# VITA-Group/Open-L2O

Measured on NVIDIA H100. Metric: coordinate-updates/sec (N_params x unroll_steps), higher is better.
Workload: dtype f32

## Files before the change

include/l2o_b200.h:

```cpp
#ifndef L2O_B200_H_
#define L2O_B200_H_

#include <stddef.h>
#include <stdint.h>

#ifdef __cplusplus
extern "C" {
#endif

#define L2O_OK 0
#define L2O_E_INVALID (-1)
#define L2O_E_UNSUPPORTED (-2)
#define L2O_E_CUDA (-3)
#define L2O_E_NOMEM (-4)

#define L2O_PRE_IDENTITY 0
#define L2O_PRE_LOGSIGN 1
#define L2O_PRE_FC 2

#define L2O_OPT_NONE 0
#define L2O_OPT_RASTRIGIN_SEP 1
#define L2O_OPT_QUADRATIC_DIAG 2
#define L2O_OPT_QUADRATIC_BATCH 3

// ... 40 lines not shown
  const float* in_seq;
  int32_t opt_kind;
  const float* opt_a;
  const float* opt_b;
  float opt_alpha;
  float opt_fscale;
  float* x;
  float* state;
  float* ckpt;
  float* m;
  float* v;
  float beta1, beta2;
  int32_t step0;
  float* g_rec;
  float* feat_rec;
  double* fx;
  float* delta_seq;
  const float* labels;
  double* imit_loss;
  int64_t n_total;
  int32_t opt_group;
} l2o_unroll_args;

typedef struct {
  int64_t n;
  int32_t T;
  const float* theta;
  const float* in_seq;
  const float* ckpt;
  const float* g_rec;
  const float* labels;
  int64_t n_total;
  double* dtheta;
  const float* delta_seq;
  float* scratch;
} l2o_bwd_args;

int l2o_net_create(l2o_handle* out, const l2o_net_desc* desc);
void l2o_net_destroy(l2o_handle h);
int l2o_net_set_engine(l2o_handle h, int32_t engine);
int64_t l2o_theta_count(l2o_handle h);
int64_t l2o_state_floats(l2o_handle h);
int l2o_workspace_bytes(l2o_handle h, int64_t n, int32_t T, size_t* fwd_bytes, size_t* bwd_bytes);

typedef struct {
  float* d_state;
  float* lam;
} l2o_bwd_carry;

int l2o_step(l2o_handle h, const l2o_step_args* a, void* stream);
int l2o_unroll_fwd(l2o_handle h, const l2o_unroll_args* a, void* stream);
int l2o_unroll_bwd(l2o_handle h, const l2o_bwd_args* a, void* stream);
int l2o_unroll_bwd_carry(l2o_handle h, const l2o_bwd_args* a, const l2o_bwd_carry* c, void* stream);

int l2o_adam_step(float* theta, const double* dtheta, float* m, float* v, int64_t n, int32_t k, float lr,
                  float beta1, float beta2, float eps, void* stream);

int l2o_log_and_sign(const float* g, float* out, int64_t n, float k, void* stream);

typedef struct l2o_dense* l2o_dense_handle;
typedef struct {
  int32_t n_layers;
  int32_t hidden[2];
  int32_t n_in;
  int32_t preprocess;
  float logsign_k;
  int32_t n_out;
  float scale;
  int32_t tanh_output;
} l2o_dense_desc;
typedef struct {
  int64_t rows;
  const float* theta;
  const float* in;
  const float* state_in;
  float* state_out;
  float* x;
  float* delta;
} l2o_dense_step_args;
typedef struct {
  int64_t rows;
  int32_t T;
  const float* theta;
  const float* in_seq;
  const float* ckpt;
  const float* g_rec;
  const float* labels;
  int64_t n_total;
  double* dtheta;
} l2o_dense_bwd_args;
int l2o_dense_create(l2o_dense_handle* out, const l2o_dense_desc* desc);
void l2o_dense_destroy(l2o_dense_handle h);
int64_t l2o_dense_theta_count(l2o_dense_handle h);
int64_t l2o_dense_state_floats(l2o_dense_handle h);
int l2o_dense_step(l2o_dense_handle h, const l2o_dense_step_args* a, void* stream);
int l2o_dense_unroll_bwd(l2o_dense_handle h, const l2o_dense_bwd_args* a, void* stream);

typedef struct {
  int32_t batch, m, n;
  const float* A;
  const float* y;
  const float* x;
  const float* scale;
  float l1;
  float* g;
  double* f;
// ... 130 lines not shown
```

open_l2o_b200/_lib.py:

```python
from __future__ import annotations

import ctypes as C
import os
import subprocess
import sys

_HERE = os.path.dirname(os.path.abspath(__file__))
_ROOT = os.path.dirname(_HERE)
CSRC = os.path.join(_HERE, "csrc")
LIB_PATH = os.environ.get("L2O_LIB") or os.path.join(CSRC, "libl2o_b200.so")
INCLUDE = os.path.join(_ROOT, "include")

L2O_OK, L2O_E_INVALID, L2O_E_UNSUPPORTED, L2O_E_CUDA, L2O_E_NOMEM = 0, -1, -2, -3, -4
PRE_IDENTITY, PRE_LOGSIGN, PRE_FC = 0, 1, 2
OPT_NONE, OPT_RASTRIGIN_SEP, OPT_QUADRATIC_DIAG, OPT_QUADRATIC_BATCH = 0, 1, 2, 3
ENGINE_AUTO, ENGINE_FFMA, ENGINE_TC = 0, 1, 2

EXPORTS = [
    "l2o_net_create", "l2o_net_destroy", "l2o_net_set_engine", "l2o_theta_count", "l2o_state_floats", "l2o_workspace_bytes",
    "l2o_step", "l2o_unroll_fwd", "l2o_unroll_bwd", "l2o_unroll_bwd_carry", "l2o_adam_step", "l2o_log_and_sign", "l2o_lasso_grad",
    "l2o_dense_create", "l2o_dense_destroy", "l2o_dense_theta_count", "l2o_dense_state_floats", "l2o_dense_step",
    "l2o_dense_unroll_bwd",
    "l2o_launch_count", "l2o_status_string", "l2o_last_cuda_error", "l2o_version",
    "l2o_hrnn_create", "l2o_hrnn_destroy", "l2o_hrnn_theta_count", "l2o_hrnn_state_floats", "l2o_hrnn_coords",
    "l2o_hrnn_workspace_bytes", "l2o_hrnn_init_state", "l2o_hrnn_prepare", "l2o_hrnn_step",
    "l2o_hrnn_set_global_sizes", "l2o_hrnn_reduce_layout", "l2o_hrnn_prepare_local", "l2o_hrnn_prepare_finish",
    "l2o_hrnn_step_local", "l2o_hrnn_step_finish", "l2o_hrnn_coord_bwd", "l2o_hrnn_workspace_layout",
    "l2o_crnn_theta_count", "l2o_crnn_state_floats", "l2o_crnn_step", "l2o_crnn_bwd",
    "l2o_tadam_theta_count", "l2o_tadam_state_floats", "l2o_tadam_step", "l2o_tadam_bwd", "l2o_lrsgd_step",
    "l2o_lrsgd_bwd",
]


class NetDesc(C.Structure):
    _fields_ = [("n_layers", C.c_int32), ("hidden", C.c_int32 * 2), ("preprocess", C.c_int32),
                ("n_in", C.c_int32), ("fc_dim", C.c_int32), ("logsign_k", C.c_float), ("scale", C.c_float),
                ("tanh_output", C.c_int32)]


_fp = C.c_void_p


class StepArgs(C.Structure):
    _fields_ = [("n", C.c_int64), ("theta", _fp), ("in0", _fp), ("in1", _fp), ("m", _fp), ("v", _fp),
                ("beta1", C.c_float), ("beta2", C.c_float), ("p", C.c_float), ("state_in", _fp),
                ("state_out", _fp), ("x", _fp), ("delta", _fp), ("feat_out", _fp), ("step_ptr", _fp), ("t_offset", C.c_int32),
                ("reuse_weights", C.c_int32)]


class UnrollArgs(C.Structure):
    _fields_ = [("n", C.c_int64), ("T", C.c_int32), ("theta", _fp), ("in_seq", _fp), ("opt_kind", C.c_int32),
                ("opt_a", _fp), ("opt_b", _fp), ("opt_alpha", C.c_float), ("opt_fscale", C.c_float), ("x", _fp),
                ("state", _fp), ("ckpt", _fp), ("m", _fp), ("v", _fp), ("beta1", C.c_float), ("beta2", C.c_float),
                ("step0", C.c_int32), ("g_rec", _fp), ("feat_rec", _fp), ("fx", _fp), ("delta_seq", _fp),
                ("labels", _fp), ("imit_loss", _fp), ("n_total", C.c_int64), ("opt_group", C.c_int32)]


class BwdArgs(C.Structure):
    _fields_ = [("n", C.c_int64), ("T", C.c_int32), ("theta", _fp), ("in_seq", _fp), ("ckpt", _fp), ("g_rec", _fp),
                ("labels", _fp), ("n_total", C.c_int64), ("dtheta", _fp), ("delta_seq", _fp), ("scratch", _fp)]


class BwdCarry(C.Structure):
    _fields_ = [("d_state", _fp), ("lam", _fp)]


class LassoArgs(C.Structure):
    _fields_ = [("batch", C.c_int32), ("m", C.c_int32), ("n", C.c_int32), ("A", _fp), ("y", _fp), ("x", _fp),
                ("scale", _fp), ("l1", C.c_float), ("g", _fp), ("f", _fp)]


class DenseDesc(C.Structure):
    _fields_ = [("n_layers", C.c_int32), ("hidden", C.c_int32 * 2), ("n_in", C.c_int32), ("preprocess", C.c_int32),
# ... 85 lines not shown
            return None
        cmd = ["nvcc"] + NVCC_FLAGS + ["-c", "-o", obj, tu]
        if verbose:
            print(" ".join(cmd), file=sys.stderr)
        r = subprocess.run(cmd, capture_output=True, text=True)
        if r.returncode != 0:
            raise L2OError("nvcc failed for %s:\n%s%s" % (tu, r.stdout, r.stderr))
        return obj

    with ThreadPoolExecutor(max_workers=max(1, min(len(jobs), os.cpu_count() or 1))) as ex:
        rebuilt = [o for o in ex.map(compile_one, jobs) if o]
    objs = [j[1] for j in jobs]
    if rebuilt or not os.path.exists(LIB_PATH) or os.path.getmtime(LIB_PATH) < max(os.path.getmtime(o) for o in objs):
        cmd = ["nvcc"] + ARCH + ["-shared", "-o", LIB_PATH] + objs
        if verbose:
            print(" ".join(cmd), file=sys.stderr)
        r = subprocess.run(cmd, capture_output=True, text=True)
        if r.returncode != 0:
            raise L2OError("link failed:\n" + r.stdout + r.stderr)
    return LIB_PATH


_lib = None


def lib():
    global _lib
    if _lib is not None:
        return _lib
    if not os.path.exists(LIB_PATH):
        raise L2OError(f"{LIB_PATH} not found - run `python -c 'import __graft_entry__ as g; g.build()'` "
                       "(there is no CPU/PyTorch fallback)")
    L = C.CDLL(LIB_PATH)
    L.l2o_net_create.argtypes = [C.POINTER(C.c_void_p), C.POINTER(NetDesc)]
    L.l2o_net_create.restype = C.c_int
    L.l2o_net_destroy.argtypes = [C.c_void_p]
    L.l2o_net_destroy.restype = None
    L.l2o_net_set_engine.argtypes = [C.c_void_p, C.c_int32]
    L.l2o_net_set_engine.restype = C.c_int
    L.l2o_theta_count.argtypes = [C.c_void_p]
    L.l2o_theta_count.restype = C.c_int64
    L.l2o_state_floats.argtypes = [C.c_void_p]
    L.l2o_state_floats.restype = C.c_int64
    L.l2o_workspace_bytes.argtypes = [C.c_void_p, C.c_int64, C.c_int32, C.POINTER(C.c_size_t), C.POINTER(C.c_size_t)]
    L.l2o_workspace_bytes.restype = C.c_int
    L.l2o_step.argtypes = [C.c_void_p, C.POINTER(StepArgs), C.c_void_p]
    L.l2o_step.restype = C.c_int
    L.l2o_unroll_fwd.argtypes = [C.c_void_p, C.POINTER(UnrollArgs), C.c_void_p]
    L.l2o_unroll_fwd.restype = C.c_int
    L.l2o_unroll_bwd.argtypes = [C.c_void_p, C.POINTER(BwdArgs), C.c_void_p]
    L.l2o_unroll_bwd.restype = C.c_int
    L.l2o_unroll_bwd_carry.argtypes = [C.c_void_p, C.POINTER(BwdArgs), C.POINTER(BwdCarry), C.c_void_p]
    L.l2o_unroll_bwd_carry.restype = C.c_int
    L.l2o_adam_step.argtypes = [C.c_void_p, C.c_void_p, C.c_void_p, C.c_void_p, C.c_int64, C.c_int32, C.c_float,
                                C.c_float, C.c_float, C.c_float, C.c_void_p]
    L.l2o_adam_step.restype = C.c_int
    L.l2o_log_and_sign.argtypes = [C.c_void_p, C.c_void_p, C.c_int64, C.c_float, C.c_void_p]
    L.l2o_log_and_sign.restype = C.c_int
    L.l2o_lasso_grad.argtypes = [C.POINTER(LassoArgs), C.c_void_p]
    L.l2o_lasso_grad.restype = C.c_int
    L.l2o_dense_create.argtypes = [C.POINTER(C.c_void_p), C.POINTER(DenseDesc)]
    L.l2o_dense_create.restype = C.c_int
    L.l2o_dense_destroy.argtypes = [C.c_void_p]
    L.l2o_dense_destroy.restype = None
    for name in ("l2o_dense_theta_count", "l2o_dense_state_floats"):
        getattr(L, name).argtypes = [C.c_void_p]
        getattr(L, name).restype = C.c_int64
    L.l2o_dense_step.argtypes = [C.c_void_p, C.POINTER(DenseStepArgs), C.c_void_p]
    L.l2o_dense_step.restype = C.c_int
    L.l2o_dense_unroll_bwd.argtypes = [C.c_void_p, C.POINTER(DenseBwdArgs), C.c_void_p]
    L.l2o_dense_unroll_bwd.restype = C.c_int
    L.l2o_launch_count.argtypes = []
    L.l2o_launch_count.restype = C.c_int64
    L.l2o_hrnn_create.argtypes = [C.POINTER(C.c_void_p), C.POINTER(C.c_int64), C.c_int32]
    L.l2o_hrnn_create.restype = C.c_int
    L.l2o_hrnn_destroy.argtypes = [C.c_void_p]
    L.l2o_hrnn_destroy.restype = None
    L.l2o_hrnn_theta_count.argtypes = []
    L.l2o_hrnn_theta_count.restype = C.c_int64
    L.l2o_hrnn_state_floats.argtypes = []
    L.l2o_hrnn_state_floats.restype = C.c_int64
    for name in ("l2o_hrnn_coords", "l2o_hrnn_workspace_bytes"):
        getattr(L, name).argtypes = [C.c_void_p]
        getattr(L, name).restype = C.c_int64
    L.l2o_hrnn_set_global_sizes.argtypes = [C.c_void_p, C.POINTER(C.c_int64)]
    L.l2o_hrnn_set_global_sizes.restype = C.c_int
    L.l2o_hrnn_reduce_layout.argtypes = [C.c_void_p, C.POINTER(C.c_int64), C.POINTER(C.c_int64), C.POINTER(C.c_int64)]
    L.l2o_hrnn_reduce_layout.restype = C.c_int
    L.l2o_hrnn_coord_bwd.argtypes = [C.c_void_p, C.POINTER(HrnnBwdArgs), C.c_void_p]
    L.l2o_hrnn_coord_bwd.restype = C.c_int
    L.l2o_hrnn_workspace_layout.argtypes = [C.c_void_p, C.POINTER(C.c_int64)]
    L.l2o_hrnn_workspace_layout.restype = C.c_int
    for name in ("l2o_hrnn_init_state", "l2o_hrnn_prepare", "l2o_hrnn_step", "l2o_hrnn_prepare_local",
                 "l2o_hrnn_prepare_finish", "l2o_hrnn_step_local", "l2o_hrnn_step_finish"):
        getattr(L, name).argtypes = [C.c_void_p, C.POINTER(HrnnArgs), C.c_void_p]
        getattr(L, name).restype = C.c_int
    for name in ("l2o_crnn_theta_count", "l2o_crnn_state_floats"):
        getattr(L, name).argtypes = []
        getattr(L, name).restype = C.c_int64
    L.l2o_crnn_step.argtypes = [C.POINTER(CrnnStepArgs), C.c_void_p]
    L.l2o_crnn_step.restype = C.c_int
    L.l2o_crnn_bwd.argtypes = [C.POINTER(CrnnBwdArgs), C.c_void_p]
    L.l2o_crnn_bwd.restype = C.c_int
    for name in ("l2o_tadam_theta_count", "l2o_tadam_state_floats"):
        getattr(L, name).argtypes = []
        getattr(L, name).restype = C.c_int64
# ... 19 lines not shown
```

open_l2o_b200/csrc/cwlstm_tc.cuh:

```cuda
#pragma once
#include "cwlstm_common.cuh"

namespace l2o {
namespace tc {

constexpr int kH = 20;
constexpr int kN = 4 * kH;
constexpr int kTile = 64;
constexpr int kU = 5;
constexpr int kFwdWG = 3;
constexpr int kFwdThreads = 128 * kFwdWG;
template <int N>
struct IC {
  static constexpr int value = N;
};

template <class C>
struct Geo {
  static constexpr bool FC = C::FC;
  static constexpr int ColH1 = FC ? 24 : 4, ColH2 = FC ? 44 : 24;
  static constexpr int ColOne = FC ? 20 : C::F;
  static constexpr int KB = FC ? 8 : 6;
  static constexpr int L1Lo = 0, L1Hi = FC ? 6 : 3;
  static constexpr int L2Lo = FC ? 2 : 0, L2Hi = KB;
// ... 217 lines not shown
    mma_rs<N>(d, f.hi[kb], bl + o, 1u);
    mma_rs<N>(d, f.hi[kb], bh + o, 1u);
  }
}

__host__ __device__ constexpr int acc_idx(int s, int g, int rh) { return 4 * (2 * s + (g >> 1)) + 2 * rh + (g & 1); }

constexpr float kLog2e = 1.4426950408889634f;
__device__ __forceinline__ void lstm_point_fwd(float zi, float zj, float zf, float zo, float& c, float& h) {
  const float Ei = ex2_approx(fminf(-kLog2e * zi, 40.f));
  const float Ej = ex2_approx(fminf(-2.f * kLog2e * zj, 40.f));
  const float Qf = 1.0f + ex2_approx(fminf(fmaf(-kLog2e, zf, -kLog2e), 40.f));
  const float Pij = (1.0f + Ei) * (1.0f + Ej);
  const float cn = fmaf(c, Pij, (1.0f - Ej) * Qf) * rcp_approx(Pij * Qf);
  c = cn;
  const float Ec = ex2_approx(fminf(-2.f * kLog2e * cn, 63.f));
  const float Eo = ex2_approx(fminf(-kLog2e * zo, 63.f));
  h = (1.0f - Ec) * rcp_approx((1.0f + Ec) * (1.0f + Eo));
}
__device__ __forceinline__ float elu_fast(float av) {
  const float em = ex2_approx(kLog2e * av) - 1.0f;
  const float ep = av * fmaf(av, fmaf(av, fmaf(av, 1.0f / 24.0f, 1.0f / 6.0f), 0.5f), 1.0f);
  return av > 0.f ? av : (av > -0.0625f ? ep : em);
}

__device__ __forceinline__ void load5(const float* __restrict__ p, int q, float* v) {
#pragma unroll
  for (int s = 0; s < kU; ++s) v[s] = p[5 * q + s];
}
__device__ __forceinline__ void store5(float* __restrict__ p, int q, const float* v) {
#pragma unroll
  for (int s = 0; s < kU; ++s) p[5 * q + s] = v[s];
}
__device__ __forceinline__ float quad_sum(float v) {
  v += __shfl_xor_sync(0xffffffffu, v, 1);
  return v + __shfl_xor_sync(0xffffffffu, v, 2);
}
__device__ __forceinline__ float from_row(float v, int lane, int rh) {
  return __shfl_sync(0xffffffffu, v, (lane & ~3) | rh);
}

struct FwdExtra {
  const int32_t* step_ptr;
  int32_t t_offset;
  float p_fixed;
};

template <class C>
struct SmemF {
  float img[Geo<C>::FwdFloats];
  float wo[kH + 4];
  float win[64];
  uint64_t wbar;
  uint64_t pad;
  double fx[1];
};
template <class C>
__host__ __device__ constexpr size_t adamc_offset(int T) {
  return (sizeof(SmemF<C>) + (size_t)(T + 1) * sizeof(double) + 15) & ~(size_t)15;
}
template <class C>
__host__ __device__ constexpr size_t fwd_smem_bytes(int T) {
  return adamc_offset<C>(T) + (C::FC ? (size_t)T * 2 * sizeof(float) : 0);
}

template <class C>
__global__ void __launch_bounds__(kFwdThreads, 1) unroll_fwd_kernel(l2o_unroll_args a, NetRt rt, const float* __restrict__ img,
                                                                     float* __restrict__ state_out, FwdExtra ex) {
  using G = Geo<C>;
  extern __shared__ __align__(128) unsigned char smem_raw[];
  SmemF<C>& S = *reinterpret_cast<SmemF<C>*>(smem_raw);
  const int T = a.T;
  const int64_t n = a.n;
  const bool in_kernel_opt = a.opt_kind != L2O_OPT_NONE;
  const bool want_fx = in_kernel_opt && a.fx != nullptr;
  const bool adam_mode = C::NIN == 2 && a.m != nullptr;
  float* adamc = reinterpret_cast<float*>(smem_raw + adamc_offset<C>(T));

  if (want_fx)
    for (int t = threadIdx.x; t <= T; t += blockDim.x) S.fx[t] = 0.0;
  if (threadIdx.x < kH) S.wo[threadIdx.x] = a.theta[C::O_WO + threadIdx.x];
  if (threadIdx.x == kH) S.wo[kH] = a.theta[C::O_BO];
  if constexpr (C::FC) {
    static_assert(!C::FC || C::NIN == 2, "fc nets here are RNNprop nets (two inputs)");
    if (threadIdx.x >= 32 && threadIdx.x < 92) S.win[threadIdx.x - 32] = a.theta[C::O_WIN + threadIdx.x - 32];
    if (adam_mode) {
      const int step0 = ex.step_ptr ? *ex.step_ptr + ex.t_offset : a.step0;
      for (int t = threadIdx.x; t < T; t += blockDim.x) {
        const float p = (ex.step_ptr == nullptr && ex.p_fixed > 0.f) ? ex.p_fixed : (float)(step0 + t);
        adamc[2 * t] = 1.0f - powf(a.beta1, p);
        adamc[2 * t + 1] = 1.0f - powf(a.beta2, p);
      }
    }
  }
  if (threadIdx.x == 0) {
    mbar_init(&S.wbar, 1);
    fence_barrier_init();
  }
  __syncthreads();
  stage_image(S.img, img, G::FwdFloats * 4, &S.wbar);

  const int wg = threadIdx.x >> 7, warp = (threadIdx.x >> 5) & 3, lane = threadIdx.x & 31;
  const int g = lane >> 2, q = lane & 3, own = q & 1;
  const uint64_t b1h = img_desc(S.img, kN), b1l = img_desc(S.img + G::B1Floats, kN);
  const uint64_t b2h = img_desc(S.img + 2 * G::B1Floats, kN), b2l = img_desc(S.img + 2 * G::B1Floats + G::B2Floats, kN);
  const int64_t ntiles = (n + kTile - 1) / kTile;
  const int64_t slot = n * C::SF;
  const float bo = S.wo[kH];
  float wo[kU];
#pragma unroll
  for (int s = 0; s < kU; ++s) wo[s] = S.wo[5 * q + s];
  double imit = 0.0;
  float d[kN / 2];
#pragma unroll
  for (int k = 0; k < kN / 2; ++k) d[k] = 0.f;

  for (int64_t tile = (int64_t)blockIdx.x * kFwdWG + wg; tile < ntiles; tile += (int64_t)gridDim.x * kFwdWG) {
    const int64_t r0 = tile * kTile + warp * 16 + g;
    const int64_t row[2] = {r0, r0 + 8};
    const bool act[2] = {row[0] < n, row[1] < n};
    const int64_t io = own ? row[1] : row[0];
    const bool oact = io < n;
    const bool writer = q < 2 && oact;
    Frag<G::KB> A;
    A.zero();
    float c1[2][kU], c2[2][kU];
#pragma unroll
    for (int rh = 0; rh < 2; ++rh) {
      float h1[kU] = {0.f, 0.f, 0.f, 0.f, 0.f}, h2[kU] = {0.f, 0.f, 0.f, 0.f, 0.f};
#pragma unroll
      for (int s = 0; s < kU; ++s) { c1[rh][s] = 0.f; c2[rh][s] = 0.f; }
      if (act[rh]) {
        const int64_t i = row[rh];
        load5(a.state + i * kH, q, h1);
        load5(a.state + (n + i) * kH, q, c1[rh]);
        load5(a.state + 2 * n * kH + i * kH, q, h2);
        load5(a.state + 2 * n * kH + (n + i) * kH, q, c2[rh]);
        if (a.ckpt) {
          store5(a.ckpt + i * kH, q, h1);
          store5(a.ckpt + (n + i) * kH, q, c1[rh]);
          store5(a.ckpt + 2 * n * kH + i * kH, q, h2);
          store5(a.ckpt + 2 * n * kH + (n + i) * kH, q, c2[rh]);
        }
        if (T == 0 && state_out != a.state) {
          store5(state_out + i * kH, q, h1);
          store5(state_out + (n + i) * kH, q, c1[rh]);
          store5(state_out + 2 * n * kH + i * kH, q, h2);
          store5(state_out + 2 * n * kH + (n + i) * kH, q, c2[rh]);
        }
      }
      A.template put_vec<G::ColH1>(rh, h1);
      A.template put_vec<G::ColH2>(rh, h2);
    }
    if constexpr (G::FC) {
      A.template put<G::ColOne>(0, q == 0 ? 1.0f : 0.f);
      A.template put<G::ColOne>(1, q == 0 ? 1.0f : 0.f);
    }
    float x = 0.f, oa = 0.f, ob = 0.f, am = 0.f, av = 0.f;
    if (oact) {
      if (a.x) x = a.x[io];
      if (in_kernel_opt) { oa = a.opt_a[io]; ob = a.opt_b[io]; }
      if (adam_mode) { am = a.m[io]; av = a.v[io]; }
    }

    for (int t = 0; t < T; ++t) {
      float fval = 0.f, raw0 = 0.f, raw1 = 0.f;
      if (oact) {
        if (in_kernel_opt) {
          optimizee_eval(a.opt_kind, x, oa, ob, a.opt_alpha, a.opt_fscale, fval, raw0);
          if (a.g_rec && q < 2) a.g_rec[(int64_t)t * n + io] = raw0;
        } else if (C::NIN == 2 && !adam_mode) {
          raw0 = a.in_seq[((int64_t)t * 2) * n + io];
          raw1 = a.in_seq[((int64_t)t * 2 + 1) * n + io];
        } else {
          raw0 = a.in_seq[(int64_t)t * n + io];
        }
      }
      if constexpr (G::FC) {
        if (adam_mode) {
          const float gg = raw0;
          am = a.beta1 * am + (1.0f - a.beta1) * gg;
          av = a.beta2 * av + (1.0f - a.beta2) * gg * gg;
          const float mh = am / adamc[2 * t], vh = av / adamc[2 * t + 1];
          const float den = sqrtf(vh) + 1e-8f;
          raw0 = mh / den;
          raw1 = gg / den;
        }
        if (writer && a.feat_rec) {
          a.feat_rec[((int64_t)t * 2) * n + io] = raw0;
          a.feat_rec[((int64_t)t * 2 + 1) * n + io] = raw1;
        }
#pragma unroll
        for (int rh = 0; rh < 2; ++rh) {
          const float m0 = from_row(raw0, lane, rh), m1 = from_row(raw1, lane, rh);
          float u[kU];
#pragma unroll
          for (int s = 0; s < kU; ++s) {
            const int j = 5 * q + s;
            u[s] = elu_fast(fmaf(m1, S.win[kH + j], fmaf(m0, S.win[j], S.win[2 * kH + j])));
          }
          A.template put_vec<0>(rh, u);
        }
      } else {
        float f[C::F];
        preprocess<C>(nullptr, rt, raw0, raw1, f);
#pragma unroll
        for (int rh = 0; rh < 2; ++rh) {
          float v = q == C::F ? 1.0f : 0.f;
#pragma unroll
          for (int k = 0; k < C::F; ++k) {
            const float fk = from_row(f[k], lane, rh);
            if (q == k) v = fk;
          }
          A.template put<0>(rh, v);
        }
      }
      if (want_fx) {
        const double ws = warp_sum_d(q < 2 ? (double)fval : 0.0);
        if (lane == 0) atomicAdd(&S.fx[t], ws);
      }
      wg_fence();
      mma3<kN, G::KB, G::L1Lo, G::L1Hi>(d, A, b1h, b1l);
      wg_commit();
      wg_wait<0>();
#pragma unroll
      for (int rh = 0; rh < 2; ++rh) {
        float h[kU];
#pragma unroll
        for (int s = 0; s < kU; ++s)
          lstm_point_fwd(d[acc_idx(s, 0, rh)], d[acc_idx(s, 1, rh)], d[acc_idx(s, 2, rh)], d[acc_idx(s, 3, rh)], c1[rh][s], h[s]);
        A.template put_vec<G::ColH1>(rh, h);
        if (act[rh]) {
          const int64_t i = row[rh];
          if (a.ckpt) {
            float* ck = a.ckpt + (int64_t)(t + 1) * slot;
            store5(ck + i * kH, q, h);
            store5(ck + (n + i) * kH, q, c1[rh]);
          }
          if (t == T - 1) {
            store5(state_out + i * kH, q, h);
            store5(state_out + (n + i) * kH, q, c1[rh]);
          }
        }
      }
      wg_fence();
      mma3<kN, G::KB, G::L2Lo, G::L2Hi>(d, A, b2h, b2l);
      wg_commit();
      wg_wait<0>();
      float y[2];
#pragma unroll
      for (int rh = 0; rh < 2; ++rh) {
        float h[kU];
        float yp = 0.f;
#pragma unroll
        for (int s = 0; s < kU; ++s) {
          lstm_point_fwd(d[acc_idx(s, 0, rh)], d[acc_idx(s, 1, rh)], d[acc_idx(s, 2, rh)], d[acc_idx(s, 3, rh)], c2[rh][s], h[s]);
          yp = fmaf(h[s], wo[s], yp);
        }
        A.template put_vec<G::ColH2>(rh, h);
        y[rh] = quad_sum(yp) + bo;
        if (act[rh]) {
          const int64_t i = row[rh];
          if (a.ckpt) {
            float* ck = a.ckpt + (int64_t)(t + 1) * slot + 2 * n * kH;
            store5(ck + i * kH, q, h);
            store5(ck + (n + i) * kH, q, c2[rh]);
          }
          if (t == T - 1) {
            store5(state_out + 2 * n * kH + i * kH, q, h);
            store5(state_out + 2 * n * kH + (n + i) * kH, q, c2[rh]);
          }
        }
      }
      const float yo = own ? y[1] : y[0];
      const float dl = rt.tanh_output ? tanh_acc(yo) * rt.scale : yo * rt.scale;
      x += dl;
      if (writer) {
        if (a.delta_seq) a.delta_seq[(int64_t)t * n + io] = dl;
        if (a.labels) {
          const float r = a.labels[(int64_t)t * n + io] - dl;
          imit += 0.5 * (double)r * (double)r;
        }
      }
    }
    float fval = 0.f;
    if (writer) {
      if (in_kernel_opt) {
        float gT;
        optimizee_eval(a.opt_kind, x, oa, ob, a.opt_alpha, a.opt_fscale, fval, gT);
        if (a.g_rec) a.g_rec[(int64_t)T * n + io] = gT;
      }
      if (a.x) a.x[io] = x;
      if (adam_mode) { a.m[io] = am; a.v[io] = av; }
    }
    if (want_fx) {
      const double ws = warp_sum_d((double)fval);
      if (lane == 0) atomicAdd(&S.fx[T], ws);
    }
  }
  if (a.labels && a.imit_loss) {
    const double ws = warp_sum_d(imit);
    if (lane == 0) atomicAdd(a.imit_loss, ws / (double)a.n_total);
  }
  __syncthreads();
  if (want_fx)
    for (int t = threadIdx.x; t <= T; t += blockDim.x) atomicAdd(&a.fx[t], S.fx[t]);
}

}

template <class C>
int tc_launch_fwd(const NetRt& rt, const l2o_unroll_args& a, float* img, cudaStream_t st, int sms, float* state_out = nullptr,
                  tc::FwdExtra ex = tc::FwdExtra{nullptr, 0, 0.f}, bool prep = true) {
  if (prep) tc::prep_weights_kernel<C><<<16, 256, 0, st>>>(a.theta, img, 0);
  auto k = tc::unroll_fwd_kernel<C>;
  const size_t smem = tc::fwd_smem_bytes<C>(a.T);
  if (smem > 227 * 1024) return L2O_E_INVALID;
  if (cudaFuncSetAttribute(k, cudaFuncAttributeMaxDynamicSharedMemorySize, (int)smem) != cudaSuccess) return L2O_E_CUDA;
  const int64_t ntiles = (a.n + tc::kTile - 1) / tc::kTile;
  const int64_t ctas = (ntiles + tc::kFwdWG - 1) / tc::kFwdWG;
  const int grid = (int)(ctas < sms ? ctas : sms);
  k<<<grid, tc::kFwdThreads, smem, st>>>(a, rt, img, state_out ? state_out : a.state, ex);
  return cudaGetLastError() == cudaSuccess ? L2O_OK : L2O_E_CUDA;
}

}
```

open_l2o_b200/csrc/l2o_capi.cu:

```cuda
#include <cuda_runtime.h>

#include <atomic>
#include <cmath>
#include <cstdio>
#include <new>

#include "l2o_internal.h"

namespace {
std::atomic<int64_t> g_launches{0};
thread_local char g_cuda_err[256] = "";

int find_cfg(const l2o_net_desc& d) {
  const int h1 = d.n_layers >= 1 ? d.hidden[0] : 0;
  const int h2 = d.n_layers >= 2 ? d.hidden[1] : 0;
  const int f = d.preprocess == L2O_PRE_FC ? d.fc_dim : (d.preprocess == L2O_PRE_LOGSIGN ? 2 * d.n_in : d.n_in);
#define X(id, PRE, NIN, F, H1, H2) \
  if (d.preprocess == PRE && d.n_in == NIN && f == F && h1 == H1 && h2 == H2) return id;
  L2O_FOR_EACH_CFG(X)
#undef X
  return -1;
}

__global__ void adam_kernel(float* __restrict__ theta, const double* __restrict__ dtheta, float* __restrict__ m,
// ... 80 lines not shown
  h->engine = engine;
  return L2O_OK;
}

int64_t l2o_theta_count(l2o_handle h) { return h ? h->n_theta : L2O_E_INVALID; }
int64_t l2o_state_floats(l2o_handle h) { return h ? h->state_floats : L2O_E_INVALID; }

int l2o_workspace_bytes(l2o_handle h, int64_t n, int32_t T, size_t* fwd_bytes, size_t* bwd_bytes) {
  if (!h || n < 0 || T < 0) return L2O_E_INVALID;
  const size_t arena = (size_t)h->state_floats * (size_t)n * sizeof(float);
  const size_t ckpt = arena * ((size_t)T + 1);
  const size_t grec = (size_t)(T + 1) * (size_t)n * sizeof(float);
  const size_t feat = h->desc.n_in == 2 ? (size_t)T * 2 * (size_t)n * sizeof(float) : 0;
  if (fwd_bytes) *fwd_bytes = arena + ckpt + grec + feat;
  const size_t fc_extra = h->cfg == 2 ? (size_t)T * (size_t)n * (1 + 20) * sizeof(float) : 0;
  if (bwd_bytes) *bwd_bytes = ckpt + grec + feat + fc_extra + (size_t)h->n_theta * sizeof(double);
  return L2O_OK;
}

int l2o_step(l2o_handle h, const l2o_step_args* a, void* stream) {
  if (!h || !a || a->n < 0 || !a->theta || !a->in0) return L2O_E_INVALID;
  if (h->state_floats > 0 && (!a->state_in || !a->state_out)) return L2O_E_INVALID;
  if (h->desc.n_in == 2 && !a->m && !a->in1) return L2O_E_INVALID;
  if ((a->m == nullptr) != (a->v == nullptr)) return L2O_E_INVALID;
  if (a->m && h->desc.n_in != 2) return L2O_E_INVALID;
  if (a->n == 0) return L2O_OK;
  cudaStream_t st = (cudaStream_t)stream;
  const bool tc_can = l2o::tc_step_ok(h, *a);
  if (h->engine == L2O_ENGINE_TC) return tc_can ? l2o::tc_step(h, *a, st) : L2O_E_UNSUPPORTED;
  if (h->engine == L2O_ENGINE_AUTO && tc_can && l2o::tc_auto_default() && a->n >= 16384) return l2o::tc_step(h, *a, st);
  return l2o::ffma_step(h, *a, st);
}

int l2o_unroll_fwd(l2o_handle h, const l2o_unroll_args* a, void* stream) {
  if (!h || !a || a->n < 0 || a->T < 0 || !a->theta) return L2O_E_INVALID;
  if (a->opt_kind == L2O_OPT_NONE && !a->in_seq && a->T > 0) return L2O_E_INVALID;
  if (a->opt_kind < L2O_OPT_NONE || a->opt_kind > L2O_OPT_QUADRATIC_BATCH) return L2O_E_INVALID;
  if (a->opt_kind == L2O_OPT_QUADRATIC_BATCH &&
      (a->opt_group < 1 || a->opt_group > 128 || a->n % a->opt_group != 0)) return L2O_E_INVALID;
  if (a->opt_kind != L2O_OPT_NONE && (!a->x || !a->opt_a || !a->opt_b)) return L2O_E_INVALID;
  if (a->opt_kind != L2O_OPT_NONE && h->desc.n_in == 2 && !a->m) return L2O_E_INVALID;
  if (h->state_floats > 0 && !a->state) return L2O_E_INVALID;
  if ((a->m == nullptr) != (a->v == nullptr)) return L2O_E_INVALID;
  if (a->m && h->desc.n_in != 2) return L2O_E_INVALID;
  if (a->labels && (!a->imit_loss || a->n_total <= 0)) return L2O_E_INVALID;
  if (a->n == 0) return L2O_OK;
  cudaStream_t st = (cudaStream_t)stream;
  const bool tc_can = l2o::tc_supported(h->cfg) && l2o::tc_fwd_ok(h, *a);
  if (h->engine == L2O_ENGINE_TC) return tc_can ? l2o::tc_unroll_fwd(h, *a, st) : L2O_E_UNSUPPORTED;
  if (h->engine == L2O_ENGINE_AUTO && tc_can && l2o::tc_auto_default()) return l2o::tc_unroll_fwd(h, *a, st);
  return l2o::ffma_unroll_fwd(h, *a, st);
}

int l2o_unroll_bwd(l2o_handle h, const l2o_bwd_args* a, void* stream) {
  if (!h || !a || a->n < 0 || a->T < 0 || !a->theta || !a->dtheta) return L2O_E_INVALID;
  if (a->T > 0 && !a->in_seq) return L2O_E_INVALID;
  if (h->state_floats > 0 && !a->ckpt) return L2O_E_INVALID;
  if (reinterpret_cast<uintptr_t>(a->ckpt) % 16 != 0) return L2O_E_INVALID;
  if (!a->g_rec && (!a->labels || a->n_total <= 0)) return L2O_E_INVALID;
  if (a->n == 0 || a->T == 0) return L2O_OK;
  cudaStream_t st = (cudaStream_t)stream;
  const bool tc_can = l2o::tc_bwd_ok(h, *a);
  if (h->engine == L2O_ENGINE_TC) return tc_can ? l2o::tc_unroll_bwd(h, *a, st) : L2O_E_UNSUPPORTED;
  if (h->engine == L2O_ENGINE_AUTO && tc_can && l2o::tc_bwd_auto_default()) return l2o::tc_unroll_bwd(h, *a, st);
  return l2o::ffma_unroll_bwd(h, *a, st);
}

int l2o_unroll_bwd_carry(l2o_handle h, const l2o_bwd_args* a, const l2o_bwd_carry* c, void* stream) {
  if (!h || !a || !c || a->n < 0 || a->T < 0 || !a->theta || !a->dtheta) return L2O_E_INVALID;
  if (a->T > 0 && !a->in_seq) return L2O_E_INVALID;
  if (h->state_floats > 0 && (!a->ckpt || !c->d_state)) return L2O_E_INVALID;
  if (reinterpret_cast<uintptr_t>(a->ckpt) % 16 != 0 || reinterpret_cast<uintptr_t>(c->d_state) % 16 != 0)
    return L2O_E_INVALID;
  if (!c->lam) return L2O_E_INVALID;
  if (!a->g_rec && (!a->labels || a->n_total <= 0)) return L2O_E_INVALID;
  if (a->labels) return L2O_E_UNSUPPORTED;
  if (a->n == 0 || a->T == 0) return L2O_OK;
  cudaStream_t st = (cudaStream_t)stream;
  const bool tc_can = l2o::tc_bwd_ok(h, *a);
  if (h->engine == L2O_ENGINE_TC) return tc_can ? l2o::tc_unroll_bwd(h, *a, st, c) : L2O_E_UNSUPPORTED;
  if (h->engine == L2O_ENGINE_AUTO && tc_can && l2o::tc_bwd_auto_default()) return l2o::tc_unroll_bwd(h, *a, st, c);
  return l2o::ffma_unroll_bwd(h, *a, st, c);
}

int l2o_adam_step(float* theta, const double* dtheta, float* m, float* v, int64_t n, int32_t k, float lr, float beta1,
                  float beta2, float eps, void* stream) {
  if (!theta || !dtheta || !m || !v || n < 0 || k < 1) return L2O_E_INVALID;
  if (n == 0) return L2O_OK;
  const double lr_t = (double)lr * std::sqrt(1.0 - std::pow((double)beta2, k)) / (1.0 - std::pow((double)beta1, k));
  const int block = 256;
  adam_kernel<<<(int)((n + block - 1) / block), block, 0, (cudaStream_t)stream>>>(theta, dtheta, m, v, n, (float)lr_t,
                                                                                 beta1, beta2, eps);
  l2o::count_launch();
  L2O_CUDA_TRY(cudaGetLastError());
  return L2O_OK;
}

int l2o_log_and_sign(const float* g, float* out, int64_t n, float k, void* stream) {
  if (!g || !out || n < 0) return L2O_E_INVALID;
  if (n == 0) return L2O_OK;
  const int block = 256;
  log_and_sign_kernel<<<(int)((n + block - 1) / block), block, 0, (cudaStream_t)stream>>>(g, out, n, k,
                                                                                         (float)std::exp((double)k));
  l2o::count_launch();
  L2O_CUDA_TRY(cudaGetLastError());
  return L2O_OK;
// ... 20 lines not shown
```

open_l2o_b200/csrc/l2o_internal.h:

```cpp
#pragma once
#include <cuda_runtime.h>

#include "cwlstm_common.cuh"
#include "l2o_b200.h"

#define L2O_FOR_EACH_CFG(X)               \
  X(0, L2O_PRE_IDENTITY, 1, 1, 20, 20)    \
  X(1, L2O_PRE_LOGSIGN, 1, 2, 20, 20)     \
  X(2, L2O_PRE_FC, 2, 20, 20, 20)         \
  X(3, L2O_PRE_IDENTITY, 1, 1, 0, 0)      \
  X(4, L2O_PRE_IDENTITY, 1, 1, 1, 0)      \
  X(5, L2O_PRE_IDENTITY, 1, 1, 1, 1)      \
  X(6, L2O_PRE_IDENTITY, 1, 1, 2, 3)

struct l2o_net {
  l2o_net_desc desc;
  int cfg;
  int engine;
  int64_t n_theta;
  int64_t state_floats;
  l2o::NetRt rt;
  float* tc_img;
  int tc_img_dev;
  int tc_img_mode;
};

namespace l2o {
int set_cuda_error(cudaError_t e, const char* where);
void count_launch(int n = 1);
int device_sms();

inline bool overlaps_any(const void* p, size_t bytes, const void* const* q, const size_t* qbytes, int nq) {
  const uintptr_t a = (uintptr_t)p;
  for (int k = 0; k < nq; ++k) {
    const uintptr_t b = (uintptr_t)q[k];
    if (b && a < b + qbytes[k] && b < a + bytes) return true;
  }
  return false;
}

int ffma_step(const l2o_net* h, const l2o_step_args& a, cudaStream_t st);
int ffma_unroll_fwd(const l2o_net* h, const l2o_unroll_args& a, cudaStream_t st);
int ffma_unroll_bwd(const l2o_net* h, const l2o_bwd_args& a, cudaStream_t st, const l2o_bwd_carry* c = nullptr);

bool tc_supported(int cfg);
void tc_release_image(l2o_net* h);
bool tc_fwd_ok(const l2o_net* h, const l2o_unroll_args& a);
int tc_unroll_fwd(l2o_net* h, const l2o_unroll_args& a, cudaStream_t st);
bool tc_step_ok(const l2o_net* h, const l2o_step_args& a);
int tc_step(l2o_net* h, const l2o_step_args& a, cudaStream_t st);
bool tc_auto_default();
bool tc_bwd_auto_default();
bool tc_bwd_ok(const l2o_net* h, const l2o_bwd_args& a);
int tc_unroll_bwd(l2o_net* h, const l2o_bwd_args& a, cudaStream_t st, const l2o_bwd_carry* c = nullptr);
}

#define L2O_CUDA_TRY(expr)                                              \
  do {                                                                  \
    cudaError_t e__ = (expr);                                           \
    if (e__ != cudaSuccess) return l2o::set_cuda_error(e__, #expr);     \
  } while (0)
```

open_l2o_b200/csrc/l2o_tc.cu:

```cuda
#include "cwlstm_ffma.cuh"
#include "cwlstm_tc.cuh"
#include "cwlstm_tc_bwd.cuh"
#include <cstdlib>
#include <mutex>
#include <utility>
#include <vector>
#include "l2o_internal.h"

namespace l2o {
bool tc_supported(int cfg) { return cfg == 0 || cfg == 1 || cfg == 2; }
bool tc_fwd_ok(const l2o_net* h, const l2o_unroll_args& a) {
  if (a.opt_kind == L2O_OPT_QUADRATIC_BATCH) return false;
  if (h->cfg == 2) return true;
  return a.m == nullptr && a.feat_rec == nullptr;
}
static bool tc_auto_env() {
  static const bool on = !(std::getenv("L2O_TC_AUTO") != nullptr && std::getenv("L2O_TC_AUTO")[0] == '0');
  return on;
}
bool tc_auto_default() { return tc_auto_env(); }
bool tc_bwd_auto_default() { return tc_auto_env(); }

namespace {
struct ImgPool {
// ... 70 lines not shown
  return tc_supported(h->cfg) && a.m == nullptr && a.in1 == nullptr && a.feat_out == nullptr;
}

int tc_step(l2o_net* h, const l2o_step_args& s, cudaStream_t st) {
  if (!tc_step_ok(h, s)) return L2O_E_UNSUPPORTED;
  int rc = ensure_image(h);
  if (rc) return rc;
  const int sms = device_sms();
  if (sms <= 0) return L2O_E_CUDA;
  l2o_unroll_args a{};
  a.n = s.n;
  a.T = 1;
  a.theta = s.theta;
  a.in_seq = s.in0;
  a.opt_kind = L2O_OPT_NONE;
  a.x = s.x;
  a.state = const_cast<float*>(s.state_in);
  a.delta_seq = s.delta;
  a.m = s.m;
  a.v = s.v;
  a.beta1 = s.beta1;
  a.beta2 = s.beta2;
  a.step0 = 1;
  a.feat_rec = s.feat_out;
  const tc::FwdExtra ex{s.step_ptr, s.t_offset, s.step_ptr ? 0.f : s.p};
  rc = L2O_E_UNSUPPORTED;
  const bool prep = !(s.reuse_weights && h->tc_img_mode == 0);
  if (h->cfg == 0) rc = tc_launch_fwd<Cfg<L2O_PRE_IDENTITY, 1, 1, 20, 20>>(h->rt, a, h->tc_img, st, sms, s.state_out, ex, prep);
  if (h->cfg == 1) rc = tc_launch_fwd<Cfg<L2O_PRE_LOGSIGN, 1, 2, 20, 20>>(h->rt, a, h->tc_img, st, sms, s.state_out, ex, prep);
  if (h->cfg == 2) rc = tc_launch_fwd<Cfg<L2O_PRE_FC, 2, 20, 20, 20>>(h->rt, a, h->tc_img, st, sms, s.state_out, ex, prep);
  if (rc == L2O_OK) count_launch(prep ? 2 : 1);
  h->tc_img_mode = 0;
  if (rc == L2O_E_CUDA) return set_cuda_error(cudaGetLastError(), "tc_step launch");
  return rc;
}

int tc_unroll_fwd(l2o_net* h, const l2o_unroll_args& a, cudaStream_t st) {
  if (!tc_supported(h->cfg) || !tc_fwd_ok(h, a)) return L2O_E_UNSUPPORTED;
  {
    int rc0 = ensure_image(h);
    if (rc0) return rc0;
  }
  const int sms = device_sms();
  if (sms <= 0) return L2O_E_CUDA;
  int rc = L2O_E_UNSUPPORTED;
  if (h->cfg == 0) rc = tc_launch_fwd<Cfg<L2O_PRE_IDENTITY, 1, 1, 20, 20>>(h->rt, a, h->tc_img, st, sms);
  if (h->cfg == 1) rc = tc_launch_fwd<Cfg<L2O_PRE_LOGSIGN, 1, 2, 20, 20>>(h->rt, a, h->tc_img, st, sms);
  if (h->cfg == 2) rc = tc_launch_fwd<Cfg<L2O_PRE_FC, 2, 20, 20, 20>>(h->rt, a, h->tc_img, st, sms);
  if (rc == L2O_OK) count_launch(2);
  h->tc_img_mode = 0;
  if (rc == L2O_E_CUDA) return set_cuda_error(cudaGetLastError(), "tc_unroll_fwd launch");
  return rc;
}
}
```

Measured before the change: 1.845 billion.

## Add specialized full-tile tensor-core forward for DM nets with in-kernel optimizee

Templates the forward unroll kernel on a FAST flag, optimizee kind and checkpoint presence, so that when n is a multiple of the tile size and no tanh, delta, or label outputs are requested, row-bound checks and runtime branches compile away. Final state is now written once after the time loop instead of inside it under a t==T-1 test. Checkpoint and g_rec addressing becomes incremental pointers. The per-step fx reduction goes straight to global atomics instead of a shared-memory buffer, and a query entry point reports which variant would run. The cost is more kernel instantiations, and more global atomic traffic on fx.

```diff
diff --git a/include/l2o_b200.h b/include/l2o_b200.h
--- a/include/l2o_b200.h
+++ b/include/l2o_b200.h
@@ -116,6 +116,7 @@
 int l2o_unroll_fwd(l2o_handle h, const l2o_unroll_args* a, void* stream);
 int l2o_unroll_bwd(l2o_handle h, const l2o_bwd_args* a, void* stream);
 int l2o_unroll_bwd_carry(l2o_handle h, const l2o_bwd_args* a, const l2o_bwd_carry* c, void* stream);
+int l2o_tc_fwd_variant(l2o_handle h, const l2o_unroll_args* a);
 
 int l2o_adam_step(float* theta, const double* dtheta, float* m, float* v, int64_t n, int32_t k, float lr,
                   float beta1, float beta2, float eps, void* stream);
diff --git a/open_l2o_b200/_lib.py b/open_l2o_b200/_lib.py
--- a/open_l2o_b200/_lib.py
+++ b/open_l2o_b200/_lib.py
@@ -18,7 +18,7 @@
 
 EXPORTS = [
     "l2o_net_create", "l2o_net_destroy", "l2o_net_set_engine", "l2o_theta_count", "l2o_state_floats", "l2o_workspace_bytes",
-    "l2o_step", "l2o_unroll_fwd", "l2o_unroll_bwd", "l2o_unroll_bwd_carry", "l2o_adam_step", "l2o_log_and_sign", "l2o_lasso_grad",
+    "l2o_step", "l2o_unroll_fwd", "l2o_unroll_bwd", "l2o_unroll_bwd_carry", "l2o_tc_fwd_variant", "l2o_adam_step", "l2o_log_and_sign", "l2o_lasso_grad",
     "l2o_dense_create", "l2o_dense_destroy", "l2o_dense_theta_count", "l2o_dense_state_floats", "l2o_dense_step",
     "l2o_dense_unroll_bwd",
     "l2o_launch_count", "l2o_status_string", "l2o_last_cuda_error", "l2o_version",
@@ -210,6 +210,8 @@
     L.l2o_unroll_bwd.restype = C.c_int
     L.l2o_unroll_bwd_carry.argtypes = [C.c_void_p, C.POINTER(BwdArgs), C.POINTER(BwdCarry), C.c_void_p]
     L.l2o_unroll_bwd_carry.restype = C.c_int
+    L.l2o_tc_fwd_variant.argtypes = [C.c_void_p, C.POINTER(UnrollArgs)]
+    L.l2o_tc_fwd_variant.restype = C.c_int
     L.l2o_adam_step.argtypes = [C.c_void_p, C.c_void_p, C.c_void_p, C.c_void_p, C.c_int64, C.c_int32, C.c_float,
                                 C.c_float, C.c_float, C.c_float, C.c_void_p]
     L.l2o_adam_step.restype = C.c_int
diff --git a/open_l2o_b200/csrc/cwlstm_tc.cuh b/open_l2o_b200/csrc/cwlstm_tc.cuh
--- a/open_l2o_b200/csrc/cwlstm_tc.cuh
+++ b/open_l2o_b200/csrc/cwlstm_tc.cuh
@@ -293,33 +293,42 @@
   float wo[kH + 4];
   float win[64];
   uint64_t wbar;
-  uint64_t pad;
-  double fx[1];
 };
 template <class C>
-__host__ __device__ constexpr size_t adamc_offset(int T) {
-  return (sizeof(SmemF<C>) + (size_t)(T + 1) * sizeof(double) + 15) & ~(size_t)15;
+__host__ __device__ constexpr size_t adamc_offset() {
+  return (sizeof(SmemF<C>) + 15) & ~(size_t)15;
 }
 template <class C>
 __host__ __device__ constexpr size_t fwd_smem_bytes(int T) {
-  return adamc_offset<C>(T) + (C::FC ? (size_t)T * 2 * sizeof(float) : 0);
-}
-
-template <class C>
+  return adamc_offset<C>() + (C::FC ? (size_t)T * 2 * sizeof(float) : 0);
+}
+__device__ __forceinline__ double warp_sum_pairs_d(double v) {
+  v += __shfl_xor_sync(0xffffffffu, v, 16);
+  v += __shfl_xor_sync(0xffffffffu, v, 8);
+  v += __shfl_xor_sync(0xffffffffu, v, 4);
+  return v + __shfl_xor_sync(0xffffffffu, v, 1);
+}
+
+template <class C, bool FAST = false, int OPT = L2O_OPT_NONE, bool CKPT = false>
 __global__ void __launch_bounds__(kFwdThreads, 1) unroll_fwd_kernel(l2o_unroll_args a, NetRt rt, const float* __restrict__ img,
                                                                      float* __restrict__ state_out, FwdExtra ex) {
+  static_assert(!FAST || (!C::FC && OPT != L2O_OPT_NONE), "the full-tile forward is the DM nets' with an optimizee");
   using G = Geo<C>;
   extern __shared__ __align__(128) unsigned char smem_raw[];
   SmemF<C>& S = *reinterpret_cast<SmemF<C>*>(smem_raw);
   const int T = a.T;
   const int64_t n = a.n;
-  const bool in_kernel_opt = a.opt_kind != L2O_OPT_NONE;
+  const bool in_kernel_opt = FAST || a.opt_kind != L2O_OPT_NONE;
+  const int opt_kind = FAST ? OPT : a.opt_kind;
   const bool want_fx = in_kernel_opt && a.fx != nullptr;
   const bool adam_mode = C::NIN == 2 && a.m != nullptr;
-  float* adamc = reinterpret_cast<float*>(smem_raw + adamc_offset<C>(T));
-
-  if (want_fx)
-    for (int t = threadIdx.x; t <= T; t += blockDim.x) S.fx[t] = 0.0;
+  const bool has_ckpt = FAST ? CKPT : a.ckpt != nullptr;
+  const bool has_grec = FAST ? CKPT : a.g_rec != nullptr;
+  const bool tanh_out = !FAST && rt.tanh_output;
+  const bool has_delta = !FAST && a.delta_seq != nullptr;
+  const bool has_labels = !FAST && a.labels != nullptr;
+  float* adamc = reinterpret_cast<float*>(smem_raw + adamc_offset<C>());
+
   if (threadIdx.x < kH) S.wo[threadIdx.x] = a.theta[C::O_WO + threadIdx.x];
   if (threadIdx.x == kH) S.wo[kH] = a.theta[C::O_BO];
   if constexpr (C::FC) {
@@ -341,12 +350,13 @@
   __syncthreads();
   stage_image(S.img, img, G::FwdFloats * 4, &S.wbar);
 
-  const int wg = threadIdx.x >> 7, warp = (threadIdx.x >> 5) & 3, lane = threadIdx.x & 31;
+  const int wg = __shfl_sync(0xffffffffu, threadIdx.x >> 7, 0), warp = (threadIdx.x >> 5) & 3, lane = threadIdx.x & 31;
   const int g = lane >> 2, q = lane & 3, own = q & 1;
   const uint64_t b1h = img_desc(S.img, kN), b1l = img_desc(S.img + G::B1Floats, kN);
   const uint64_t b2h = img_desc(S.img + 2 * G::B1Floats, kN), b2l = img_desc(S.img + 2 * G::B1Floats + G::B2Floats, kN);
   const int64_t ntiles = (n + kTile - 1) / kTile;
   const int64_t slot = n * C::SF;
+  const int64_t nk = n * kH;
   const float bo = S.wo[kH];
   float wo[kU];
 #pragma unroll
@@ -359,10 +369,12 @@
   for (int64_t tile = (int64_t)blockIdx.x * kFwdWG + wg; tile < ntiles; tile += (int64_t)gridDim.x * kFwdWG) {
     const int64_t r0 = tile * kTile + warp * 16 + g;
     const int64_t row[2] = {r0, r0 + 8};
-    const bool act[2] = {row[0] < n, row[1] < n};
+    const bool act[2] = {FAST || row[0] < n, FAST || row[1] < n};
     const int64_t io = own ? row[1] : row[0];
-    const bool oact = io < n;
+    const bool oact = FAST || io < n;
     const bool writer = q < 2 && oact;
+    float* ck = has_ckpt ? a.ckpt + r0 * kH : nullptr;
+    float* gr = has_grec ? a.g_rec + io : nullptr;
     Frag<G::KB> A;
     A.zero();
     float c1[2][kU], c2[2][kU];
@@ -377,13 +389,14 @@
         load5(a.state + (n + i) * kH, q, c1[rh]);
         load5(a.state + 2 * n * kH + i * kH, q, h2);
         load5(a.state + 2 * n * kH + (n + i) * kH, q, c2[rh]);
-        if (a.ckpt) {
-          store5(a.ckpt + i * kH, q, h1);
-          store5(a.ckpt + (n + i) * kH, q, c1[rh]);
-          store5(a.ckpt + 2 * n * kH + i * kH, q, h2);
-          store5(a.ckpt + 2 * n * kH + (n + i) * kH, q, c2[rh]);
-        }
-        if (T == 0 && state_out != a.state) {
+        if (has_ckpt) {
+          float* p = ck + rh * 8 * kH;
+          store5(p, q, h1);
+          store5(p + nk, q, c1[rh]);
+          store5(p + 2 * nk, q, h2);
+          store5(p + 3 * nk, q, c2[rh]);
+        }
+        if (!FAST && T == 0 && state_out != a.state) {
           store5(state_out + i * kH, q, h1);
           store5(state_out + (n + i) * kH, q, c1[rh]);
           store5(state_out + 2 * n * kH + i * kH, q, h2);
@@ -399,17 +412,21 @@
     }
     float x = 0.f, oa = 0.f, ob = 0.f, am = 0.f, av = 0.f;
     if (oact) {
-      if (a.x) x = a.x[io];
+      if (FAST || a.x) x = a.x[io];
       if (in_kernel_opt) { oa = a.opt_a[io]; ob = a.opt_b[io]; }
       if (adam_mode) { am = a.m[io]; av = a.v[io]; }
     }
 
     for (int t = 0; t < T; ++t) {
+      if (has_ckpt) ck += slot;
       float fval = 0.f, raw0 = 0.f, raw1 = 0.f;
       if (oact) {
         if (in_kernel_opt) {
-          optimizee_eval(a.opt_kind, x, oa, ob, a.opt_alpha, a.opt_fscale, fval, raw0);
-          if (a.g_rec && q < 2) a.g_rec[(int64_t)t * n + io] = raw0;
+          optimizee_eval(opt_kind, x, oa, ob, a.opt_alpha, a.opt_fscale, fval, raw0);
+          if (has_grec) {
+            if (q < 2) *gr = raw0;
+            gr += n;
+          }
         } else if (C::NIN == 2 && !adam_mode) {
           raw0 = a.in_seq[((int64_t)t * 2) * n + io];
           raw1 = a.in_seq[((int64_t)t * 2 + 1) * n + io];
@@ -457,8 +474,8 @@
         }
       }
       if (want_fx) {
-        const double ws = warp_sum_d(q < 2 ? (double)fval : 0.0);
-        if (lane == 0) atomicAdd(&S.fx[t], ws);
+        const double ws = warp_sum_pairs_d(q < 2 ? (double)fval : 0.0);
+        if (lane == 0) atomicAdd(&a.fx[t], ws);
       }
       wg_fence();
       mma3<kN, G::KB, G::L1Lo, G::L1Hi>(d, A, b1h, b1l);
@@ -471,18 +488,11 @@
         for (int s = 0; s < kU; ++s)
           lstm_point_fwd(d[acc_idx(s, 0, rh)], d[acc_idx(s, 1, rh)], d[acc_idx(s, 2, rh)], d[acc_idx(s, 3, rh)], c1[rh][s], h[s]);
         A.template put_vec<G::ColH1>(rh, h);
-        if (act[rh]) {
-          const int64_t i = row[rh];
-          if (a.ckpt) {
-            float* ck = a.ckpt + (int64_t)(t + 1) * slot;
-            store5(ck + i * kH, q, h);
-            store5(ck + (n + i) * kH, q, c1[rh]);
-          }
-          if (t == T - 1) {
-            store5(state_out + i * kH, q, h);
-            store5(state_out + (n + i) * kH, q, c1[rh]);
-          }
-        }
+        if (act[rh] && has_ckpt) {
+          store5(ck + rh * 8 * kH, q, h);
+          store5(ck + nk + rh * 8 * kH, q, c1[rh]);
+        }
+        if (has_ckpt) __syncwarp();
       }
       wg_fence();
       mma3<kN, G::KB, G::L2Lo, G::L2Hi>(d, A, b2h, b2l);
@@ -500,61 +510,73 @@
         }
         A.template put_vec<G::ColH2>(rh, h);
         y[rh] = quad_sum(yp) + bo;
-        if (act[rh]) {
-          const int64_t i = row[rh];
-          if (a.ckpt) {
-            float* ck = a.ckpt + (int64_t)(t + 1) * slot + 2 * n * kH;
-            store5(ck + i * kH, q, h);
-            store5(ck + (n + i) * kH, q, c2[rh]);
-          }
-          if (t == T - 1) {
-            store5(state_out + 2 * n * kH + i * kH, q, h);
-            store5(state_out + 2 * n * kH + (n + i) * kH, q, c2[rh]);
-          }
-        }
+        if (act[rh] && has_ckpt) {
+          store5(ck + 2 * nk + rh * 8 * kH, q, h);
+          store5(ck + 3 * nk + rh * 8 * kH, q, c2[rh]);
+        }
+        if (has_ckpt) __syncwarp();
       }
       const float yo = own ? y[1] : y[0];
-      const float dl = rt.tanh_output ? tanh_acc(yo) * rt.scale : yo * rt.scale;
+      const float dl = tanh_out ? tanh_acc(yo) * rt.scale : __fmul_rn(yo, rt.scale);
       x += dl;
       if (writer) {
-        if (a.delta_seq) a.delta_seq[(int64_t)t * n + io] = dl;
-        if (a.labels) {
+        if (has_delta) a.delta_seq[(int64_t)t * n + io] = dl;
+        if (has_labels) {
           const float r = a.labels[(int64_t)t * n + io] - dl;
           imit += 0.5 * (double)r * (double)r;
         }
+      }
+    }
+    if (FAST || T > 0) {
+#pragma unroll
+      for (int rh = 0; rh < 2; ++rh) {
+        if (!act[rh]) continue;
+        float h1[kU], h2[kU];
+#pragma unroll
+        for (int s = 0; s < kU; ++s) {
+          h1[s] = A.get_at(G::ColH1 + 4 * s, rh);
+          h2[s] = A.get_at(G::ColH2 + 4 * s, rh);
+        }
+        float* p = state_out + row[rh] * kH;
+        store5(p, q, h1);
+        store5(p + nk, q, c1[rh]);
+        store5(p + 2 * nk, q, h2);
+        store5(p + 3 * nk, q, c2[rh]);
       }
     }
     float fval = 0.f;
     if (writer) {
       if (in_kernel_opt) {
         float gT;
-        optimizee_eval(a.opt_kind, x, oa, ob, a.opt_alpha, a.opt_fscale, fval, gT);
-        if (a.g_rec) a.g_rec[(int64_t)T * n + io] = gT;
-      }
-      if (a.x) a.x[io] = x;
+        optimizee_eval(opt_kind, x, oa, ob, a.opt_alpha, a.opt_fscale, fval, gT);
+        if (has_grec) *gr = gT;
+      }
+      if (FAST || a.x) a.x[io] = x;
       if (adam_mode) { a.m[io] = am; a.v[io] = av; }
     }
     if (want_fx) {
-      const double ws = warp_sum_d((double)fval);
-      if (lane == 0) atomicAdd(&S.fx[T], ws);
-    }
-  }
-  if (a.labels && a.imit_loss) {
+      const double ws = warp_sum_pairs_d((double)fval);
+      if (lane == 0) atomicAdd(&a.fx[T], ws);
+    }
+  }
+  if (has_labels && a.imit_loss) {
     const double ws = warp_sum_d(imit);
     if (lane == 0) atomicAdd(a.imit_loss, ws / (double)a.n_total);
   }
-  __syncthreads();
-  if (want_fx)
-    for (int t = threadIdx.x; t <= T; t += blockDim.x) atomicAdd(&a.fx[t], S.fx[t]);
-}
-
-}
-
-template <class C>
-int tc_launch_fwd(const NetRt& rt, const l2o_unroll_args& a, float* img, cudaStream_t st, int sms, float* state_out = nullptr,
-                  tc::FwdExtra ex = tc::FwdExtra{nullptr, 0, 0.f}, bool prep = true) {
-  if (prep) tc::prep_weights_kernel<C><<<16, 256, 0, st>>>(a.theta, img, 0);
-  auto k = tc::unroll_fwd_kernel<C>;
+}
+
+}
+
+inline bool tc_fwd_fast(bool fc, const NetRt& rt, const l2o_unroll_args& a, const float* state_out) {
+  return !fc && (a.opt_kind == L2O_OPT_RASTRIGIN_SEP || a.opt_kind == L2O_OPT_QUADRATIC_DIAG) && a.n > 0 &&
+         a.n % tc::kTile == 0 && a.T > 0 && (state_out == nullptr || state_out == a.state) && a.x != nullptr &&
+         (a.ckpt == nullptr) == (a.g_rec == nullptr) && !rt.tanh_output && a.delta_seq == nullptr && a.labels == nullptr;
+}
+
+template <class C, bool FAST, int OPT, bool CKPT>
+int tc_run_fwd(const NetRt& rt, const l2o_unroll_args& a, float* img, cudaStream_t st, int sms, float* state_out,
+               tc::FwdExtra ex) {
+  auto k = tc::unroll_fwd_kernel<C, FAST, OPT, CKPT>;
   const size_t smem = tc::fwd_smem_bytes<C>(a.T);
   if (smem > 227 * 1024) return L2O_E_INVALID;
   if (cudaFuncSetAttribute(k, cudaFuncAttributeMaxDynamicSharedMemorySize, (int)smem) != cudaSuccess) return L2O_E_CUDA;
@@ -565,4 +587,21 @@
   return cudaGetLastError() == cudaSuccess ? L2O_OK : L2O_E_CUDA;
 }
 
-}
+template <class C>
+int tc_launch_fwd(const NetRt& rt, const l2o_unroll_args& a, float* img, cudaStream_t st, int sms, float* state_out = nullptr,
+                  tc::FwdExtra ex = tc::FwdExtra{nullptr, 0, 0.f}, bool prep = true) {
+  if (prep) tc::prep_weights_kernel<C><<<16, 256, 0, st>>>(a.theta, img, 0);
+  if constexpr (!C::FC) {
+    if (tc_fwd_fast(false, rt, a, state_out)) {
+      constexpr int R = L2O_OPT_RASTRIGIN_SEP, Q = L2O_OPT_QUADRATIC_DIAG;
+      if (a.opt_kind == R)
+        return a.ckpt ? tc_run_fwd<C, true, R, true>(rt, a, img, st, sms, state_out, ex)
+                      : tc_run_fwd<C, true, R, false>(rt, a, img, st, sms, state_out, ex);
+      return a.ckpt ? tc_run_fwd<C, true, Q, true>(rt, a, img, st, sms, state_out, ex)
+                    : tc_run_fwd<C, true, Q, false>(rt, a, img, st, sms, state_out, ex);
+    }
+  }
+  return tc_run_fwd<C, false, L2O_OPT_NONE, false>(rt, a, img, st, sms, state_out, ex);
+}
+
+}
diff --git a/open_l2o_b200/csrc/l2o_capi.cu b/open_l2o_b200/csrc/l2o_capi.cu
--- a/open_l2o_b200/csrc/l2o_capi.cu
+++ b/open_l2o_b200/csrc/l2o_capi.cu
@@ -156,6 +156,11 @@
   return l2o::ffma_unroll_fwd(h, *a, st);
 }
 
+int l2o_tc_fwd_variant(l2o_handle h, const l2o_unroll_args* a) {
+  if (!h || !a) return L2O_E_INVALID;
+  return l2o::tc_fwd_variant(h, *a);
+}
+
 int l2o_unroll_bwd(l2o_handle h, const l2o_bwd_args* a, void* stream) {
   if (!h || !a || a->n < 0 || a->T < 0 || !a->theta || !a->dtheta) return L2O_E_INVALID;
   if (a->T > 0 && !a->in_seq) return L2O_E_INVALID;
diff --git a/open_l2o_b200/csrc/l2o_internal.h b/open_l2o_b200/csrc/l2o_internal.h
--- a/open_l2o_b200/csrc/l2o_internal.h
+++ b/open_l2o_b200/csrc/l2o_internal.h
@@ -47,6 +47,7 @@
 void tc_release_image(l2o_net* h);
 bool tc_fwd_ok(const l2o_net* h, const l2o_unroll_args& a);
 int tc_unroll_fwd(l2o_net* h, const l2o_unroll_args& a, cudaStream_t st);
+int tc_fwd_variant(const l2o_net* h, const l2o_unroll_args& a);
 bool tc_step_ok(const l2o_net* h, const l2o_step_args& a);
 int tc_step(l2o_net* h, const l2o_step_args& a, cudaStream_t st);
 bool tc_auto_default();
diff --git a/open_l2o_b200/csrc/l2o_tc.cu b/open_l2o_b200/csrc/l2o_tc.cu
--- a/open_l2o_b200/csrc/l2o_tc.cu
+++ b/open_l2o_b200/csrc/l2o_tc.cu
@@ -146,4 +146,9 @@
   if (rc == L2O_E_CUDA) return set_cuda_error(cudaGetLastError(), "tc_unroll_fwd launch");
   return rc;
 }
+
+int tc_fwd_variant(const l2o_net* h, const l2o_unroll_args& a) {
+  if (!tc_supported(h->cfg) || !tc_fwd_ok(h, a)) return L2O_E_UNSUPPORTED;
+  return tc_fwd_fast(h->cfg == 2, h->rt, a, nullptr) ? 1 : 0;
 }
+}
```

After: 1.909 billion (median of 6 runs). 1.04x the previous value.
